# zobront/mythril

Hardware: AMD Instinct MI355X
Metric: candidate-assignment evals/sec (higher is better)
Workload: dtype u256 (u32 limbs); 1 GPU; C5 (BASELINE.json configs[4], per-GPU shard), exhaustive search; candidates_per_gpu_step=4194304, engine=jit (mwj_9cb5b0f4019c115a), jit_split=False, rccl_world=1, candidate_begin=0

## Files before the change

### mythril_amd/csrc/mw_alu.h

```cpp
#pragma once
#include <stdint.h>
#include <hip/hip_runtime.h>

#define MW_HD __host__ __device__ __attribute__((always_inline)) inline

#if defined(__HIP_DEVICE_COMPILE__)
#define MW_ANY(c) (__ballot(c) != 0ull)
#else
#define MW_ANY(c) (c)
#endif
#if defined(MW_DIV_NO_HINTS)
#define MW_RARE(c) (c)
#define MW_USUAL(c) (c)
#else
#define MW_RARE(c) __builtin_expect(!!(c), 0)
#define MW_USUAL(c) __builtin_expect(!!(c), 1)
#endif

namespace mw {
typedef uint32_t u32;
typedef uint64_t u64;

MW_HD u32 addc(u32 a, u32 b, u32& c) {
  u32 co;
// ... 392 lines not shown
#else
  const u32 n = y[7] ? 0u : y[6] ? 1u : y[5] ? 2u : y[4] ? 3u : y[3] ? 4u : y[2] ? 5u : y[1] ? 6u : 7u;
#pragma unroll
  for (int st = 0; st < 3; ++st) {
    const int m = 1 << st;
    const bool c = (n >> st) & 1u;
#pragma unroll
    for (int k = 7; k >= 0; --k) v[k] = c ? (k >= m ? v[k - m] : 0u) : v[k];
#pragma unroll
    for (int k = 15; k >= 0; --k) u[k] = c ? (k >= m ? u[k - m] : 0u) : u[k];
  }
#endif
  u32 w[9], lo[7], qq[8];
#pragma unroll
  for (int k = 0; k < 9; ++k) w[k] = u[7 + k];
#pragma unroll
  for (int k = 0; k < 7; ++k) lo[k] = u[k];
#pragma unroll
  for (int k = 0; k < 8; ++k) qq[k] = 0u;
#pragma unroll 1
  for (int it = 0; it < 8; ++it) {
    u32 qd = 0u;
    if (MW_ANY(w[8] != 0u || w[7] >= v[7])) {
      if (dc) dc->steps += 1u;
      qd = qdigit_est3(w[8], w[7], w[6], v[7], v[6]);
      u32 carry = 0, br = 0;
#pragma unroll
      for (int k = 0; k < 8; ++k) {
        const u64 p = (u64)qd * v[k] + carry;
        carry = (u32)(p >> 32);
        w[k] = subb(w[k], (u32)p, br);
      }
      u32 hi = w[8] - carry - br;
      while (MW_RARE(MW_ANY(hi != 0u))) {
        if (hi != 0u) {
          u32 c = 0;
#pragma unroll
          for (int k = 0; k < 8; ++k) w[k] = addc(w[k], v[k], c);
          hi += c;
          qd -= 1u;
        }
      }
      w[8] = 0u;
    }
#pragma unroll
    for (int k = 7; k > 0; --k) qq[k] = qq[k - 1];
    qq[0] = qd;
    if (it < 7) {
#pragma unroll
      for (int k = 8; k > 0; --k) w[k] = w[k - 1];
      w[0] = lo[6];
#pragma unroll
      for (int k = 6; k > 0; --k) lo[k] = lo[k - 1];
      lo[0] = 0u;
    }
  }
#pragma unroll
  for (int k = 0; k < 8; ++k) {
    q[k] = qq[k];
    u[k] = w[k];
    u[k + 8] = 0u;
  }
#if defined(MW_GEN_ROLLED_SHIFT)
#pragma unroll 1
  for (int st = 0; st < 7; ++st) {
    const bool c = n > (u32)st;
    if (!MW_ANY(c)) break;
#pragma unroll
    for (int k = 0; k < 7; ++k) u[k] = c ? u[k + 1] : u[k];
    u[7] = c ? 0u : u[7];
  }
#else
#pragma unroll
  for (int st = 0; st < 3; ++st) {
    const int m = 1 << st;
    const bool c = (n >> st) & 1u;
#pragma unroll
    for (int k = 0; k < 8; ++k) u[k] = c ? (k + m < 16 ? u[k + m] : 0u) : u[k];
  }
#endif
  copy8(r, u);
}

MW_HD void neg8(const u32 a[8], u32 r[8]) {
  u32 br = 0;
#pragma unroll
  for (int k = 0; k < 8; ++k) r[k] = subb(0u, a[k], br);
}
MW_HD void cneg8(u32 a[8], bool c, u32 w) {
  u32 br = 0;
#pragma unroll
  for (int k = 0; k < 8; ++k) {
    const u32 t = subb(0u, a[k], br);
    a[k] = c ? t : a[k];
  }
  canon(a, w);
}

MW_HD void wdiv(int kind, u32 x[8], u32 y[8], u32 w, u32 r[8], DivCount* dc = nullptr) {
  bool sa = false, sb = false;
  if (kind >= 2) {
    sa = signbit8(x, w);
    sb = signbit8(y, w);
    cneg8(x, sa, w);
    cneg8(y, sb, w);
  }
  const bool yz = is_zero8(y);
  y[0] |= yz ? 1u : 0u;
  u32 q[8];
  udivrem8(x, y, q, r, dc);
  if (yz) {
#pragma unroll
    for (int k = 0; k < 8; ++k) {
      q[k] = limb_mask(w, k);
      r[k] = x[k];
    }
  }
  switch (kind) {
    case 0:
      copy8(r, q);
      break;
    case 1:
      break;
    case 2:
      copy8(r, q);
      cneg8(r, sa != sb, w);
      break;
    case 3:
      cneg8(r, sa, w);
      break;
    default: {
      const bool uz = is_zero8(r);
      if (yz) y[0] = 0u;
      cneg8(y, sb, w);
      const bool negu = sa;
      cneg8(r, negu, w);
      const bool addt = !uz && (sa != sb);
      u32 c = 0;
#pragma unroll
      for (int k = 0; k < 8; ++k) {
        const u32 t = addc(r[k], y[k], c);
        r[k] = addt ? t : r[k];
      }
      break;
    }
  }
  canon(r, w);
}

MW_HD u32 n_sext(u32 a, u32 wfrom) {
  if (wfrom >= 32) return a;
  u32 s = (a >> (wfrom - 1)) & 1u;
  return s ? (a | ~nmask(wfrom)) : a;
}
MW_HD u32 n_div(int kind, u32 a, u32 b, u32 w) {
  u32 m = nmask(w);
  bool sa = false, sb = false;
  u32 x = a, y = b;
  if (kind >= 2) {
    sa = (a >> (w - 1)) & 1u;
    sb = (b >> (w - 1)) & 1u;
    x = sa ? ((0u - a) & m) : a;
    y = sb ? ((0u - b) & m) : b;
  }
  u32 q, rm;
  if (y == 0) {
    q = m;
    rm = x;
  } else {
    q = x / y;
    rm = x - q * y;
  }
  u32 r;
  switch (kind) {
    case 0: r = q; break;
    case 1: r = rm; break;
    case 2: r = (sa != sb) ? (0u - q) : q; break;
    case 3: r = sa ? (0u - rm) : rm; break;
    default: {
      if (rm == 0) r = 0;
      else if (!sa && !sb) r = rm;
      else if (sa && !sb) r = (0u - rm) + b;
      else if (!sa && sb) r = rm + b;
      else r = 0u - rm;
      break;
    }
  }
  return r & m;
}
MW_HD u32 n_shl(u32 a, u32 b, u32 w) { return b >= w ? 0u : ((a << b) & nmask(w)); }
MW_HD u32 n_lshr(u32 a, u32 b, u32 w) { return b >= w ? 0u : (a >> b); }
MW_HD u32 n_ashr(u32 a, u32 b, u32 w) {
  int32_t sa = (int32_t)n_sext(a, w);
  u32 s = b >= w ? 31u : b;
  return ((u32)(sa >> s)) & nmask(w);
}
MW_HD bool n_slt(u32 a, u32 b, u32 w) { return (int32_t)n_sext(a, w) < (int32_t)n_sext(b, w); }
MW_HD bool n_sle(u32 a, u32 b, u32 w) { return (int32_t)n_sext(a, w) <= (int32_t)n_sext(b, w); }
MW_HD bool n_umulno(u32 a, u32 b, u32 w) {
  u64 p = (u64)a * b;
  return w >= 32 ? (p >> 32) == 0 : (p >> w) == 0;
}

}
```

### mythril_amd/csrc/mw_jit.h

```cpp
#pragma once
#if defined(__HIP_DEVICE_COMPILE__)
#define MW_LEAF_KEY_FENCE(k) asm volatile("" : "+s"(k))
#endif
#include "mw_alu.h"
#include "mw_isa.h"
#include "mw_leaf.h"

namespace mw {
namespace jit {
MW_HD void xor8(const u32 x[8], const u32 y[8], u32 r[8]) {
#pragma unroll
  for (int k = 0; k < 8; ++k) r[k] = x[k] ^ y[k];
}

#if defined(MW_ABLATE_ADD)
#define add8(x, y, r) ((void)xor8(x, y, r), 0u)
#define sub8(x, y, r) ((void)xor8(x, y, r), 0u)
#endif
#if defined(MW_ABLATE_MUL)
#define mul8(x, y, r) xor8(x, y, r)
#endif
MW_HD void w_add(const u32 x[8], const u32 y[8], u32 w, u32 r[8]) { add8(x, y, r); canon(r, w); }
MW_HD void w_sub(const u32 x[8], const u32 y[8], u32 w, u32 r[8]) { sub8(x, y, r); canon(r, w); }
MW_HD void w_mul(const u32 x[8], const u32 y[8], u32 w, u32 r[8]) { mul8(x, y, r); canon(r, w); }
// ... 44 lines not shown
      "v_addc_co_u32_e64 %[c], %[s2], %[c], 0, %[s2]\n"
      "v_addc_co_u32_e64 %[c], %[s0], %[c], 0, %[s0]\n"
      "v_addc_co_u32_e64 %[c], %[s1], %[c], 0, %[s1]\n"
      : [p] "+v"(p), [c] "=&v"(c), [s0] "=&s"(s0), [s1] "=&s"(s1), [s2] "=&s"(s2)
      : [a0] "v"(a[0]), [a1] "v"(a[1]), [a2] "v"(a[2]), [a3] "v"(a[3]), [a4] "v"(a[4]), [b0] "v"(b[0]), [b1] "v"(b[1]), [b2] "v"(b[2]), [b3] "v"(b[3]), [b4] "v"(b[4]));
  r[4] = (u32)p;
  p = (p >> 32) | ((u64)c << 32);
  asm("v_mad_u64_u32 %[p], %[s0], %[a0], %[b5], %[p]\n"
      "v_mad_u64_u32 %[p], %[s1], %[a1], %[b4], %[p]\n"
      "v_mad_u64_u32 %[p], %[s2], %[a2], %[b3], %[p]\n"
      "v_addc_co_u32_e64 %[c], %[s0], 0, 0, %[s0]\n"
      "v_mad_u64_u32 %[p], %[s0], %[a3], %[b2], %[p]\n"
      "v_addc_co_u32_e64 %[c], %[s1], %[c], 0, %[s1]\n"
      "v_mad_u64_u32 %[p], %[s1], %[a4], %[b1], %[p]\n"
      "v_addc_co_u32_e64 %[c], %[s2], %[c], 0, %[s2]\n"
      "v_mad_u64_u32 %[p], %[s2], %[a5], %[b0], %[p]\n"
      "v_addc_co_u32_e64 %[c], %[s0], %[c], 0, %[s0]\n"
      "v_addc_co_u32_e64 %[c], %[s1], %[c], 0, %[s1]\n"
      "v_addc_co_u32_e64 %[c], %[s2], %[c], 0, %[s2]\n"
      : [p] "+v"(p), [c] "=&v"(c), [s0] "=&s"(s0), [s1] "=&s"(s1), [s2] "=&s"(s2)
      : [a0] "v"(a[0]), [a1] "v"(a[1]), [a2] "v"(a[2]), [a3] "v"(a[3]), [a4] "v"(a[4]), [a5] "v"(a[5]), [b0] "v"(b[0]), [b1] "v"(b[1]), [b2] "v"(b[2]), [b3] "v"(b[3]), [b4] "v"(b[4]), [b5] "v"(b[5]));
  r[5] = (u32)p;
  p = (p >> 32) | ((u64)c << 32);
  asm("v_mad_u64_u32 %[p], %[s0], %[a0], %[b6], %[p]\n"
      "v_mad_u64_u32 %[p], %[s1], %[a1], %[b5], %[p]\n"
      "v_mad_u64_u32 %[p], %[s2], %[a2], %[b4], %[p]\n"
      "v_mad_u64_u32 %[p], %[s0], %[a3], %[b3], %[p]\n"
      "v_mad_u64_u32 %[p], %[s1], %[a4], %[b2], %[p]\n"
      "v_mad_u64_u32 %[p], %[s2], %[a5], %[b1], %[p]\n"
      "v_mad_u64_u32 %[p], %[s0], %[a6], %[b0], %[p]\n"
      : [p] "+v"(p), [s0] "=&s"(s0), [s1] "=&s"(s1), [s2] "=&s"(s2)
      : [a0] "v"(a[0]), [a1] "v"(a[1]), [a2] "v"(a[2]), [a3] "v"(a[3]), [a4] "v"(a[4]), [a5] "v"(a[5]), [a6] "v"(a[6]), [b0] "v"(b[0]), [b1] "v"(b[1]), [b2] "v"(b[2]), [b3] "v"(b[3]), [b4] "v"(b[4]), [b5] "v"(b[5]), [b6] "v"(b[6]));
  r[6] = (u32)p;
  r[7] = (u32)(p >> 32) + a[0] * b[7] + a[1] * b[6] + a[2] * b[5] + a[3] * b[4] + a[4] * b[3] + a[5] * b[2] +
         a[6] * b[1] + a[7] * b[0];
#else
  mul8(a, b, r);
#endif
}
#if defined(MW_ABLATE_MUL)
#define mul8_cols(x, y, r) xor8(x, y, r)
#endif
MW_HD void w_mulv(const u32 x[8], const u32 y[8], u32 w, u32 r[8]) { mul8_cols(x, y, r); canon(r, w); }
MW_HD void w_and(const u32 x[8], const u32 y[8], u32 w, u32 r[8]) {
#pragma unroll
  for (int k = 0; k < 8; ++k) r[k] = x[k] & y[k];
  canon(r, w);
}
MW_HD void w_or(const u32 x[8], const u32 y[8], u32 w, u32 r[8]) {
#pragma unroll
  for (int k = 0; k < 8; ++k) r[k] = x[k] | y[k];
  canon(r, w);
}
MW_HD void w_xor(const u32 x[8], const u32 y[8], u32 w, u32 r[8]) {
#pragma unroll
  for (int k = 0; k < 8; ++k) r[k] = x[k] ^ y[k];
  canon(r, w);
}
MW_HD void w_not(const u32 x[8], u32 w, u32 r[8]) {
#pragma unroll
  for (int k = 0; k < 8; ++k) r[k] = ~x[k];
  canon(r, w);
}
#if defined(MW_ABLATE_SHIFT)
MW_HD void w_shl(const u32 x[8], const u32 y[8], u32 w, u32 r[8]) { xor8(x, y, r); }
MW_HD void w_lshr(const u32 x[8], const u32 y[8], u32 w, u32 r[8]) { xor8(x, y, r); }
MW_HD void w_ashr(const u32 x[8], const u32 y[8], u32 w, u32 r[8]) { xor8(x, y, r); }
#else
MW_HD void w_shl(const u32 x[8], const u32 y[8], u32 w, u32 r[8]) { wshl(x, y, w, r); canon(r, w); }
MW_HD void w_lshr(const u32 x[8], const u32 y[8], u32 w, u32 r[8]) { wlshr(x, y, w, r); canon(r, w); }
MW_HD void w_ashr(const u32 x[8], const u32 y[8], u32 w, u32 r[8]) { washr(x, y, w, r); canon(r, w); }
#endif
MW_HD void w_div(int kind, const u32 x[8], const u32 y[8], u32 w, u32 r[8], DivCount& dc) {
#if defined(MW_ABLATE_DIV)
  xor8(x, y, r);
  return;
#endif
  u32 a[8], b[8];
  copy8(a, x);
  copy8(b, y);
  wdiv(kind, a, b, w, r, &dc);
  canon(r, w);
}
MW_HD void w_ite(u32 c, const u32 x[8], const u32 y[8], u32 w, u32 r[8]) {
#pragma unroll
  for (int k = 0; k < 8; ++k) r[k] = c ? x[k] : y[k];
  canon(r, w);
}
MW_HD void w_shli(const u32 x[8], u32 imm, u32 w, u32 r[8]) { shl8(x, imm, r); canon(r, w); }
MW_HD void w_lshri(const u32 x[8], u32 imm, u32 w, u32 r[8]) { shr8(x, imm, 0u, r); canon(r, w); }
MW_HD void w_zextn(u32 v, u32 w, u32 r[8]) {
  zero8(r);
  r[0] = v;
  canon(r, w);
}
MW_HD void w_sext(const u32 x[8], u32 imm, u32 w, u32 r[8]) {
  copy8(r, x);
  sext8(r, imm);
  canon(r, w);
}
MW_HD void w_sextn(u32 v, u32 imm, u32 w, u32 r[8]) {
  zero8(r);
  r[0] = v;
  sext8(r, imm);
  canon(r, w);
}
MW_HD void w_insn(const u32 x[8], u32 v, u32 imm, u32 w, u32 r[8]) {
  u32 y[8];
  zero8(y);
  y[0] = v;
  shl8(y, imm, r);
#pragma unroll
  for (int k = 0; k < 8; ++k) r[k] |= x[k];
  canon(r, w);
}
MW_HD void w_mov(const u32 x[8], u32 w, u32 r[8]) {
  copy8(r, x);
  canon(r, w);
}

MW_HD u32 n_extractw(const u32 x[8], u32 imm, u32 w) {
  u32 r[8];
  shr8(x, imm, 0u, r);
  return r[0] & nmask(w);
}
MW_HD u32 n_ult(const u32 x[8], const u32 y[8]) { return ult8(x, y) ? 1u : 0u; }
MW_HD u32 n_ule(const u32 x[8], const u32 y[8]) { return ult8(y, x) ? 0u : 1u; }
MW_HD u32 n_scmp(const u32 x_[8], const u32 y_[8], u32 w, bool le) {
  u32 x[8], y[8];
#pragma unroll
  for (int k = 0; k < 8; ++k) {
    const int bit = (int)w - 1 - 32 * k;
    const u32 m = (bit >= 0 && bit < 32) ? (1u << bit) : 0u;
    x[k] = x_[k] ^ m;
    y[k] = y_[k] ^ m;
  }
  return (le ? !ult8(y, x) : ult8(x, y)) ? 1u : 0u;
}
MW_HD u32 n_eq(const u32 x[8], const u32 y[8]) { return eq8(x, y) ? 1u : 0u; }
MW_HD u32 n_umulno(const u32 x[8], const u32 y[8], u32 w) {
  u32 lo[8], hi[8];
  mulhi8(x, y, lo, hi);
  u32 ov = 0;
#pragma unroll
  for (int k = 0; k < 8; ++k) ov |= (lo[k] & ~limb_mask(w, k)) | hi[k];
  return ov ? 0u : 1u;
}
MW_HD u32 n_addc(const u32 x[8], const u32 y[8], u32 w) {
  u32 r[8];
  const u32 c = add8(x, y, r);
  u32 bit = 0;
#pragma unroll
  for (int k = 0; k < 8; ++k) {
    const int b = (int)w - 32 * k;
    bit |= (b >= 0 && b < 32) ? ((r[k] >> b) & 1u) : 0u;
  }
  return (w >= 256) ? c : bit;
}

MW_HD u32 nn_add(u32 a, u32 b, u32 w) { return (a + b) & nmask(w); }
MW_HD u32 nn_sub(u32 a, u32 b, u32 w) { return (a - b) & nmask(w); }
MW_HD u32 nn_mul(u32 a, u32 b, u32 w) { return (a * b) & nmask(w); }
MW_HD u32 nn_not(u32 a, u32 w) { return (~a) & nmask(w); }
MW_HD u32 nn_shli(u32 a, u32 imm, u32 w) { return (imm >= 32 ? 0u : (a << imm)) & nmask(w); }
MW_HD u32 nn_lshri(u32 a, u32 imm, u32 w) { return (imm >= 32 ? 0u : (a >> imm)) & nmask(w); }
MW_HD u32 nn_sext(u32 a, u32 imm, u32 w) { return n_sext(a, imm) & nmask(w); }
// ... 73 lines not shown
  do {                                                     \
    asm volatile("" : "+s"(ctl));                          \
    if (__builtin_expect((ctl & MW_JIT_NEVER) != 0u, 0))   \
      asm volatile("s_nop 0");                             \
  } while (0)
#else
#define JIT_SPLIT() ((void)ctl)
#endif

typedef bool (*body_fn)(const u32* __restrict__, u64, u64, bool, u32, u32*, u64, u64, DivCount&);

#define MW_JIT_FIRST 1u
#define MW_JIT_LAST 2u

#if !defined(MW_JIT_HOST)
template <body_fn BODY>
__device__ __attribute__((always_inline)) inline void search(const u32* __restrict__ pool, u64 seed, u64 begin,
                                                             u64 count, u64 chunk0, u32 flags,
                                                             u64* __restrict__ out_min, u64* __restrict__ counter,
                                                             u32* __restrict__ verdict, u32* __restrict__ alivebuf,
                                                             u32 stage) {
  const u64 base = begin + (chunk0 + blockIdx.x) * 256;
  if ((flags & MW_FLAG_STOP_AFTER_HIT) && stage == (MW_JIT_FIRST | MW_JIT_LAST)) {
    const u64 m = __hip_atomic_load(out_min, __ATOMIC_RELAXED, __HIP_MEMORY_SCOPE_AGENT);
    if (m <= base) return;
  }
  const u32 lane = threadIdx.x & 63u;
  const u64 cand = base + threadIdx.x;
  const bool valid = cand < begin + count;
  bool in = valid;
  if (!(stage & MW_JIT_FIRST) && valid) in = alivebuf[cand - begin] != 0u;
  DivCount dc;
  const bool ok = BODY(pool, seed, cand, in, flags, nullptr, 0, 0, dc);
  const u64 nvalid = (u64)__popcll(__ballot(valid));
  const bool counting = !(flags & MW_FLAG_NO_COUNT);
  counter += MW_CTR_STRIPE_WORDS * (1u + (blockIdx.x & (MW_CTR_STRIPES - 1u)));
  if (counting && lane == 0 && nvalid)
    add_div_counts(counter, dc, nvalid);
  if (!(stage & MW_JIT_LAST)) {
    if (valid) alivebuf[cand - begin] = ok ? 1u : 0u;
    return;
  }
  if (verdict && valid) verdict[cand - begin] = ok ? 1u : 0u;
  const u64 hit = __ballot(ok);
  if (hit) {
    const u32 first = (u32)__ffsll((unsigned long long)hit) - 1u;
    if (lane == first && cand < __hip_atomic_load(out_min, __ATOMIC_RELAXED, __HIP_MEMORY_SCOPE_AGENT))
      atomicMin((unsigned long long*)out_min, (unsigned long long)cand);
  }
  if (counting && lane == 0 && nvalid) atomicAdd((unsigned long long*)counter, (unsigned long long)nvalid);
}

#ifndef MW_JIT_WAVES
#define MW_JIT_WAVES 2
#endif
#define MW_JIT_KERNEL(NAME, SUFFIX, BODY, EARLY)                                                     \
  extern "C" __global__ __launch_bounds__(256, MW_JIT_WAVES) void NAME##SUFFIX(                      \
      const mw::u32* __restrict__ pool, mw::u64 seed, mw::u64 begin, mw::u64 count, mw::u64 chunk0,  \
      mw::u32 flags, mw::u64* __restrict__ out_min, mw::u64* __restrict__ counter,                   \
      mw::u32* __restrict__ verdict, mw::u32* __restrict__ alivebuf, mw::u32 stage) {                \
    mw::jit::search<BODY<EARLY>>(pool, seed, begin, count, chunk0, flags, out_min, counter, verdict, \
                                 alivebuf, stage);                                                   \
  }
#define MW_JIT_SIG(NAME, SIG) extern "C" __device__ const mw::u64 NAME##_sig = SIG;
#define MW_JIT_PART(NAME, K, N)                                \
  extern "C" __device__ const mw::u32 NAME##_part = K;         \
  extern "C" __device__ const mw::u32 NAME##_nparts = N;
#else
#define MW_JIT_KERNEL(NAME, SUFFIX, BODY, EARLY)
#define MW_JIT_SIG(NAME, SIG)
#define MW_JIT_PART(NAME, K, N)
#endif

#if defined(MW_JIT_HOST)
#define MW_JIT_HOST_ENTRY(NAME, BODY)                                                                \
  extern "C" int NAME##_host(const mw::u32* pool, mw::u64 seed, mw::u64 begin, mw::u64 count,        \
                             mw::u32 early, mw::u32* verdict, mw::u32* trace) {                      \
    for (mw::u64 i = 0; i < count; ++i) {                                                            \
      mw::DivCount ds;                                                                               \
      verdict[i] = (early ? BODY<true>(pool, seed, begin + i, true, 0u, trace, count, i, ds)             \
                          : BODY<false>(pool, seed, begin + i, true, 0u, trace, count, i, ds)) ? 1u : 0u; \
    }                                                                                                \
    return 0;                                                                                        \
  }
#else
#define MW_JIT_HOST_ENTRY(NAME, BODY)
#endif

}
}
```

### mythril_amd/jit.py

```python
from __future__ import annotations

import hashlib
import os
import subprocess
import sys
import tempfile
import time
from pathlib import Path
from typing import Dict, List, Optional, Sequence, Tuple

import numpy as np

from . import isa
from .compiler import Const, MInsn, Program, VReg, compile_program

ROOT = Path(__file__).resolve().parent.parent
CSRC = ROOT / "mythril_amd" / "csrc"
ARCH = os.environ.get("MW_OFFLOAD_ARCH", "gfx950")
HEADERS = ["mw_jit.h", "mw_alu.h", "mw_isa.h", "mw_leaf.h"]
M256 = (1 << 256) - 1
SPLIT_EVERY = 48
SPLIT_KIND = os.environ.get("MW_JIT_SPLIT", "branch")
CHECK_SYNC = os.environ.get("MW_JIT_CHECK_SYNC", "0") == "1"
CHECK_SYNC_EVERY = int(os.environ.get("MW_JIT_CHECK_SYNC_EVERY", "1"))
MUL_COLS = os.environ.get("MW_JIT_MUL_COLS", "1") == "1"
LDS_AHEAD = int(os.environ.get("MW_JIT_LDS_AHEAD", "16"))
LDS_AHEAD_W = int(os.environ.get("MW_JIT_LDS_AHEAD_W", "0"))
LDS_AHEAD_STOP = int(os.environ.get("MW_JIT_LDS_AHEAD_STOP", "500"))
LDS_REUSE = int(os.environ.get("MW_JIT_LDS_REUSE", "96"))
M32 = 0xFFFFFFFF

_WBIN = {"W_ADD": "w_add", "W_SUB": "w_sub", "W_MUL": "w_mul", "W_AND": "w_and", "W_OR": "w_or",
         "W_XOR": "w_xor", "W_SHL": "w_shl", "W_LSHR": "w_lshr", "W_ASHR": "w_ashr"}
_DIV = {"UDIV": 0, "UREM": 1, "SDIV": 2, "SREM": 3, "SMOD": 4}
_NBIN = {"N_ADD": "jit::nn_add({a}, {b}, {w})", "N_SUB": "jit::nn_sub({a}, {b}, {w})",
         "N_MUL": "jit::nn_mul({a}, {b}, {w})", "N_AND": "({a} & {b})", "N_OR": "({a} | {b})",
         "N_XOR": "({a} ^ {b})", "N_SHL": "n_shl({a}, {b}, {w})", "N_LSHR": "n_lshr({a}, {b}, {w})",
         "N_ASHR": "n_ashr({a}, {b}, {w})", "N_ULTN": "(u32)({a} < {b})", "N_ULEN": "(u32)({a} <= {b})",
         "N_SLTN": "(u32)n_slt({a}, {b}, {w})", "N_SLEN": "(u32)n_sle({a}, {b}, {w})",
         "N_EQN": "(u32)({a} == {b})", "N_UMULNON": "(u32)n_umulno({a}, {b}, {w})",
         "N_ADDCN": "jit::nn_addc({a}, {b}, {w})"}


def _cache_dir() -> Path:
    return Path(os.environ.get("MW_JIT_CACHE", str(ROOT / "build" / "jit")))


def signature(p: Program) -> int:
    h = 0xCBF29CE484222325
    for arr in (p.code, p.consts, p.leaves, p.pool):
        a = np.ascontiguousarray(arr, dtype=np.uint32)
        h = _fnv_words(h, a)
    return h


def _fnv_words(h: int, a: np.ndarray) -> int:
    b = a.astype("<u4").view(np.uint8)
    P = 0x100000001B3
    M = (1 << 64) - 1
    for x in b.tobytes():
        h = ((h ^ x) * P) & M
    return h


def interleave_conjuncts(insns: List[MInsn], k: int) -> List[MInsn]:
    if k <= 1:
        return list(insns)
    segs: List[List[MInsn]] = []
    cur: List[MInsn] = []
    tail: List[MInsn] = []
    for ins in insns:
        if ins.op == "END":
            tail.append(ins)
            continue
        cur.append(ins)
        if ins.op == "CHECK":
            segs.append(cur)
            cur = []
    if cur:
        segs.append(cur)
    out: List[MInsn] = []
    defined = set()
    for g in range(0, len(segs), k):
        group = segs[g:g + k]
        pos = [0] * len(group)
        left = sum(len(sg) for sg in group)
        while left:
            for j, sg in enumerate(group):
                if pos[j] >= len(sg):
                    continue
                ins = sg[pos[j]]
                if any(isinstance(s_, VReg) and s_.id not in defined for s_ in ins.srcs):
                    continue
                out.append(ins)
                if ins.dst is not None:
                    defined.add(ins.dst.id)
                pos[j] += 1
                left -= 1
    return out + tail


class _Gen:

    def __init__(self, p: Program, name: str, fence_first: bool = False, lds_leaves: int = 0,
                 insns: Optional[List[MInsn]] = None, interleave: int = 1, mul_cols: Optional[bool] = None):
        self.fence_first = fence_first
        self.mul_cols = MUL_COLS if mul_cols is None else mul_cols
        self.p = p
        self.insns = interleave_conjuncts(p.machine_ir() if insns is None else insns, interleave)
        uses: Dict[int, int] = {}
        defs: Dict[int, int] = {}
        for ins in self.insns:
            if ins.op == "LEAF_W":
                defs[ins.dst.id] = ins.imm
            for s_ in ins.srcs:
                if isinstance(s_, VReg) and s_.id in defs:
                    uses[s_.id] = uses.get(s_.id, 0) + 1
        hot = sorted(uses, key=lambda v: -uses[v])[:lds_leaves]
        self.lds_slot: Dict[int, int] = {v: k for k, v in enumerate(hot)}
        self.pre: List[str] = []
        self.nl = 0
        self.name = name
        self.wconst: Dict[int, str] = {}
        self.lines: List[str] = []
        self.since_split = 0
        self.nf = 0
        self.put_at: Dict[int, int] = {}
        self.line_w: List[int] = []
        self.nchecks = 0
        self.last_reload: Dict[int, Tuple[str, int]] = {}

    def W(self, s) -> str:
        if isinstance(s, Const):
            v = s.value & M256
            n = self.wconst.get(v)
            if n is None:
                n = f"k{len(self.wconst)}"
                self.wconst[v] = n
            return n
        if s.cls != "W":
            raise ValueError("N register in a W operand")
        slot = self.lds_slot.get(s.id)
        if slot is not None:
            last = self.last_reload.get(s.id)
            if LDS_REUSE and last is not None and len(self.lines) - last[1] <= LDS_REUSE:
                return last[0]
            self.nl += 1
            self.last_reload[s.id] = (f"L{self.nl}", len(self.lines))
            self.pre.append(("R", f"u32 L{self.nl}[8]; jit::lds_get8({slot}u, L{self.nl});", s.id))
            return f"L{self.nl}"
        return f"v{s.id}"

    def N(self, s) -> str:
        if isinstance(s, Const):
            return f"{s.value & M32:#x}u"
        if s.cls != "N":
            raise ValueError("W register in an N operand")
        return f"n{s.id}"

    def leaf(self, li: int, dst: str):
        L = [int(x) for x in self.p.leaves[li * isa.LEAF_WORDS:(li + 1) * isa.LEAF_WORDS]]
        w, kind, lid, shift, bits, poff, _inrow, stride = L
        return (f"leaf_fields({w}u, {kind}u, {lid:#x}u, {shift}u, {bits}u, {poff}u, {stride}u, "
                f"pool, seed, cand, {dst});")

    def emit(self, ins) -> None:
        n0 = len(self.lines)
        self._emit(ins)
        self.line_w.extend([0] * (len(self.lines) - len(self.line_w)))
        if len(self.lines) > n0:
            self.line_w[-1] = insn_weight(ins)

    def _emit(self, ins) -> None:
        op, w, d, S, imm = ins.op, ins.width, ins.dst, ins.srcs, ins.imm
        self.since_split += 1
        if self.since_split > SPLIT_EVERY and op != "CHECK":
            self.lines.append("JIT_SPLIT();")
            self.since_split = 0
        if op == "END":
            return
        shape = isa.SHAPES[op]
        A = [self.W(s) if c == "W" else self.N(s) for s, c in zip(S, shape[1])]
        out = self.lines.append
        for x in self.pre:
            out(x)
        self.pre = []
        fence = getattr(ins, "remat", False)
        if fence or (self.fence_first and S and op not in ("CHECK", "STORE_W", "STORE_N")):
            for j, (s, c) in enumerate(zip(S, shape[1])):
                if not fence and j > 0:
                    break
                if isinstance(s, VReg):
                    self.nf += 1
                    if c == "W":
                        out(f"u32 f{self.nf}[8]; jit::fence8({A[j]}, f{self.nf});")
                        A[j] = f"f{self.nf}"
                    else:
                        out(f"const u32 f{self.nf} = jit::fence1({A[j]});")
                        A[j] = f"f{self.nf}"
        dn = None
        if d is not None:
            dn = f"v{d.id}" if d.cls == "W" else f"n{d.id}"
        if op == "CHECK":
            self.nchecks += 1
            sync = CHECK_SYNC and self.nchecks % CHECK_SYNC_EVERY == 0
            tail = "{ JIT_SPLIT(); JIT_SYNC(); }" if sync else "JIT_SPLIT();"
            out(f"alive = jit::check(alive, {A[0]}); if (EARLY) {{ if (jit::none(alive)) break; }} else {tail}")
            self.since_split = 0
        elif op == "LEAF_W" and d.id in self.lds_slot:
            out(f"{{ u32 t_[8]; {self.leaf(imm, 't_')} jit::lds_put8({self.lds_slot[d.id]}u, t_); }}")
            self.put_at[d.id] = len(self.lines)
        elif op == "LEAF_W":
            out(f"u32 {dn}[8]; {self.leaf(imm, dn)}")
        elif op == "LEAF_N":
            out(f"u32 {dn}; {{ u32 t_[8]; {self.leaf(imm, 't_')} {dn} = t_[0]; }}")
        elif op in ("STORE_W", "STORE_N"):
            row = self.p.trace_map[-imm - 1][0]
            if op == "STORE_W":
                out(f"jit::tstore(trace, tstride, tidx, {row}u, {A[0]}, 8);")
            else:
                out(f"{{ const u32 t_ = {A[0]}; jit::tstore(trace, tstride, tidx, {row}u, &t_, 1); }}")
        elif op == "MOV_W":
            out(f"u32 {dn}[8]; jit::w_mov({A[0]}, {w}u, {dn});")
        elif op == "MOV_N":
            out(f"const u32 {dn} = {A[0]};")
        elif op == "W_MUL" and self.mul_cols and all(isinstance(s, VReg) for s in S):
            out(f"u32 {dn}[8]; jit::w_mulv({A[0]}, {A[1]}, {w}u, {dn});")
        elif op in _WBIN:
            out(f"u32 {dn}[8]; jit::{_WBIN[op]}({A[0]}, {A[1]}, {w}u, {dn});")
        elif op.startswith("W_") and op[2:] in _DIV:
            out(f"u32 {dn}[8]; jit::w_div({_DIV[op[2:]]}, {A[0]}, {A[1]}, {w}u, {dn}, dsteps);")
        elif op == "W_NOT":
            out(f"u32 {dn}[8]; jit::w_not({A[0]}, {w}u, {dn});")
        elif op == "W_ITE":
            out(f"u32 {dn}[8]; jit::w_ite({A[2]}, {A[0]}, {A[1]}, {w}u, {dn});")
        elif op == "W_SHLI":
            out(f"u32 {dn}[8]; jit::w_shli({A[0]}, {imm}u, {w}u, {dn});")
        elif op == "W_LSHRI":
            out(f"u32 {dn}[8]; jit::w_lshri({A[0]}, {imm}u, {w}u, {dn});")
        elif op == "W_ZEXTN":
            out(f"u32 {dn}[8]; jit::w_zextn({A[0]}, {w}u, {dn});")
        elif op == "W_SEXT":
            out(f"u32 {dn}[8]; jit::w_sext({A[0]}, {imm}u, {w}u, {dn});")
        elif op == "W_SEXTN":
            out(f"u32 {dn}[8]; jit::w_sextn({A[0]}, {imm}u, {w}u, {dn});")
        elif op == "W_INSN":
            out(f"u32 {dn}[8]; jit::w_insn({A[0]}, {A[1]}, {imm}u, {w}u, {dn});")
        elif op == "N_EXTRACTW":
            out(f"const u32 {dn} = jit::n_extractw({A[0]}, {imm}u, {w}u);")
        elif op == "N_ULT":
            out(f"const u32 {dn} = jit::n_ult({A[0]}, {A[1]});")
        elif op == "N_ULE":
            out(f"const u32 {dn} = jit::n_ule({A[0]}, {A[1]});")
        elif op in ("N_SLT", "N_SLE"):
            le = "true" if op == "N_SLE" else "false"
            out(f"const u32 {dn} = jit::n_scmp({A[0]}, {A[1]}, {w}u, {le});")
        elif op == "N_EQ":
            out(f"const u32 {dn} = jit::n_eq({A[0]}, {A[1]});")
        elif op == "N_UMULNO":
            out(f"const u32 {dn} = jit::n_umulno({A[0]}, {A[1]}, {w}u);")
        elif op == "N_ADDC":
            out(f"const u32 {dn} = jit::n_addc({A[0]}, {A[1]}, {w}u);")
        elif op in _NBIN:
            out(f"const u32 {dn} = " + _NBIN[op].format(a=A[0], b=A[1], w=f"{w}u") + ";")
        elif op.startswith("N_") and op[2:] in _DIV:
            out(f"const u32 {dn} = n_div({_DIV[op[2:]]}, {A[0]}, {A[1]}, {w}u);")
        elif op == "N_NOT":
            out(f"const u32 {dn} = jit::nn_not({A[0]}, {w}u);")
        elif op == "N_ITE":
            out(f"const u32 {dn} = {A[2]} ? {A[0]} : {A[1]};")
        elif op == "N_SHLI":
            out(f"const u32 {dn} = jit::nn_shli({A[0]}, {imm}u, {w}u);")
        elif op == "N_LSHRI":
            out(f"const u32 {dn} = jit::nn_lshri({A[0]}, {imm}u, {w}u);")
        elif op == "N_SEXT":
            out(f"const u32 {dn} = jit::nn_sext({A[0]}, {imm}u, {w}u);")
        else:
            raise ValueError(f"jit: no emitter for {op}")

    def _place_reloads(self) -> List[str]:
        if LDS_AHEAD <= 0 and LDS_AHEAD_W <= 0:
            return [x[1] if isinstance(x, tuple) else x for x in self.lines]
        before: Dict[int, List[str]] = {}
        rest: List[Tuple[int, str]] = []
        for i, x in enumerate(self.lines):
            if isinstance(x, tuple):
                floor = self.put_at.get(x[2], -1) + 1
                if LDS_AHEAD_W > 0:
                    j, acc = i, 0
                    while j > floor and acc < LDS_AHEAD_W:
                        j -= 1
                        acc += self.line_w[j]
                elif LDS_AHEAD_STOP < (1 << 30):
                    j = i
                    while j > floor and i - j < LDS_AHEAD and self.line_w[j - 1] < LDS_AHEAD_STOP:
                        j -= 1
                else:
                    j = max(i - LDS_AHEAD, floor)
                before.setdefault(j, []).append(x[1])
            else:
                rest.append((i, x))
        out: List[str] = []
        pend = sorted(before)
        k = 0
        for i, x in rest:
            while k < len(pend) and pend[k] <= i:
                out += before[pend[k]]
                k += 1
            out.append(x)
        while k < len(pend):
            out += before[pend[k]]
            k += 1
        return out

    def body(self) -> str:
        for ins in self.insns:
            self.emit(ins)
        self.lines = self._place_reloads()
        head = [f"template <bool EARLY>",
                f"MW_HD bool {self.name}_body(const u32* __restrict__ pool, u64 seed, u64 cand, bool alive,",
                f"                             u32 ctl, u32* __restrict__ trace, u64 tstride, u64 tidx,",
                f"                             DivCount& dsteps) {{"]
        consts = []
        for v, n in self.wconst.items():
            limbs = ", ".join(f"{(v >> (32 * k)) & M32:#x}u" for k in range(8))
            consts.append(f"  const u32 {n}[8] = {{{limbs}}};")
        return "\n".join(head + consts + ["  do {"] + ["    " + x for x in self.lines] +
                         ["  } while (0);", "  return alive;", "}"])


PART_WEIGHT = 110_000
_WEIGHT = {"W_UDIV": 900, "W_UREM": 900, "W_SDIV": 950, "W_SREM": 950, "W_SMOD": 950, "W_MUL": 110,
           "W_SHL": 45, "W_LSHR": 45, "W_ASHR": 45, "LEAF_W": 200, "LEAF_N": 100, "N_ULT": 25, "N_ULE": 25,
           "N_SLT": 30, "N_SLE": 30, "N_EQ": 16, "N_UMULNO": 150, "N_ADDC": 12}


def insn_weight(ins: MInsn) -> int:
    w = _WEIGHT.get(ins.op)
    if w is not None:
        return w
    return 10 if ins.op.startswith("W_") else 3


def split_ssa(p: Program, part_weight: int = PART_WEIGHT) -> List[List[MInsn]]:
    ssa = [i for i in p.machine_ir() if i.op != "END"]
    n = len(ssa)
    total = sum(insn_weight(i) for i in ssa)
    if total <= part_weight * 1.25 or n < 2:
        return [p.machine_ir()]
    defs: Dict[int, int] = {}
    last: Dict[int, int] = {}
    for i, ins in enumerate(ssa):
        if ins.dst is not None:
            defs[ins.dst.id] = i
        for s_ in ins.srcs:
            if isinstance(s_, VReg):
                last[s_.id] = i
    delta = [0] * (n + 2)
    for vid, d in defs.items():
        if ssa[d].op.startswith("LEAF"):
            continue
        l = last.get(vid, d)
        if l > d:
            delta[d + 1] += 1
            delta[l + 1] -= 1
    cuts, acc, cross = [], 0, 0
    target = total / max(2, round(total / part_weight))
    for b in range(1, n):
        cross += delta[b]
        acc += insn_weight(ssa[b - 1])
        if acc >= target and ssa[b - 1].op == "CHECK" and cross == 0:
            cuts.append(b)
            acc = 0
    if not cuts:
        return [p.machine_ir()]
    bounds = [0] + cuts + [n]
    parts = []
    for a, b in zip(bounds, bounds[1:]):
        seg = ssa[a:b]
        inside = {ins.dst.id for ins in seg if ins.dst is not None}
        need, stack = set(), [s_.id for ins in seg for s_ in ins.srcs if isinstance(s_, VReg)]
        while stack:
            v = stack.pop()
            if v in inside or v in need:
                continue
            need.add(v)
            stack.extend(s_.id for s_ in ssa[defs[v]].srcs if isinstance(s_, VReg))
        pre = [ssa[defs[v]] for v in sorted(need, key=lambda v: defs[v])]
        parts.append(pre + seg + [MInsn("END")])
    return parts


def generate(progs: Sequence[Program], names: Sequence[str], variants: str = "xe",
             fence_first: bool = False, lds_leaves: int = 0,
             parts: Optional[Sequence[Tuple[List[MInsn], int, int]]] = None, interleave: int = 1,
             mul_cols: Optional[bool] = None) -> str:
    out = ["// generated by mythril_amd/jit.py: specialised witness-search kernels"]
    if lds_leaves:
        out.append(f"#define MW_JIT_LDS_SLOTS {lds_leaves}")
    out += ['#include "mw_jit.h"', "using namespace mw;", ""]
    if SPLIT_KIND == "sched_barrier":
        out += ["#if defined(__HIP_DEVICE_COMPILE__)", "#undef JIT_SPLIT",
                "#define JIT_SPLIT() __builtin_amdgcn_sched_barrier(0)", "#endif", ""]
    if CHECK_SYNC:
        out += ["#if defined(__HIP_DEVICE_COMPILE__)", "#define JIT_SYNC() __syncthreads()", "#else",
                "#define JIT_SYNC() ((void)0)", "#endif", ""]
    done = set()
    for k, (p, name) in enumerate(zip(progs, names)):
        if name in done:
            continue
        done.add(name)
        if not p.machine_ir():
            raise ValueError("program has no SSA machine IR (compiled by an older compiler?)")
        part = parts[k] if parts else None
        out.append(f"// program {name}: {p.n_insn} bytecode insns, {p.ops_per_eval} u32 ops/eval"
                   + (f", part {part[1]} of {part[2]}" if part else ""))
        out.append(_Gen(p, name, fence_first, lds_leaves, part[0] if part else None, interleave, mul_cols).body())
        out.append(f"MW_JIT_SIG({name}, {signature(p):#x}ull)")
        if part:
            out.append(f"MW_JIT_PART({name}, {part[1]}u, {part[2]}u)")
        if "x" in variants:
            out.append(f"MW_JIT_KERNEL({name}, _x, {name}_body, false)")
        if "e" in variants:
            out.append(f"MW_JIT_KERNEL({name}, _e, {name}_body, true)")
        out.append(f"MW_JIT_HOST_ENTRY({name}, {name}_body)")
        out.append("")
    return "\n".join(out)


def kernel_name(p: Program) -> str:
    return f"mwj_{signature(p):016x}"


def _hipcc() -> str:
    return "/opt/rocm/bin/hipcc" if os.path.exists("/opt/rocm/bin/hipcc") else "hipcc"


def _key(src: str, flags: Sequence[str]) -> str:
    h = hashlib.sha256(src.encode())
    h.update(" ".join(flags).encode())
    for hd in HEADERS:
        h.update((CSRC / hd).read_bytes())
    return h.hexdigest()[:24]


DEVICE_FLAGS = ["--genco", f"--offload-arch={ARCH}", "-O3", "-std=c++17", "-Wno-unused-variable"]
HOST_FLAGS = ["-O1", "-std=c++17", "-fPIC", "-shared", "-D__HIP_PLATFORM_AMD__", "-DMW_JIT_HOST",
              "-Wno-unused-variable"]


_USED: set = set()


def prune_cache(keep: Optional[set] = None) -> int:
    keep = _USED if keep is None else keep
    n = 0
    for f in _cache_dir().glob("*"):
        if f not in keep:
            f.unlink()
            n += 1
    return n


def _compile(src: str, flags: Sequence[str], suffix: str, ext: str) -> Tuple[Path, float]:
    cache = _cache_dir()
    cache.mkdir(parents=True, exist_ok=True)
    out = cache / f"{_key(src, flags)}{suffix}"
    _USED.add(out)
    if out.exists():
        return out, 0.0
    t0 = time.perf_counter()
    with tempfile.TemporaryDirectory() as td:
        f = Path(td) / f"k{ext}"
        f.write_text(src)
        tmp = Path(td) / ("out" + suffix)
        proc = subprocess.Popen([_hipcc(), *flags, f"-I{CSRC}", str(f), "-o", str(tmp)],
                                stdout=subprocess.PIPE, stderr=subprocess.PIPE, text=True)
        while True:
            try:
                _, err = proc.communicate(timeout=30)
                break
            except subprocess.TimeoutExpired:
                print(f"[jit] compiling {len(src) // 1024} KiB of HIP for {ARCH}: "
                      f"{time.perf_counter() - t0:.0f} s", file=sys.stderr, flush=True)
        if proc.returncode != 0:
            raise RuntimeError(f"jit compile failed:\n{err[-4000:]}")
        os.replace(tmp, out)
    return out, time.perf_counter() - t0


def is_cached(progs: Sequence[Program], variants: str = "xe", waves: int = 2, lds_leaves: int = 0,
              interleave: int = 1, mul_cols: Optional[bool] = None) -> bool:
    names = [kernel_name(p) for p in progs]
    src = generate(progs, names, variants, lds_leaves=lds_leaves, interleave=interleave, mul_cols=mul_cols)
    return (_cache_dir() / f"{_key(src, _device_flags(waves))}.hsaco").exists()


def compile_device(progs: Sequence[Program], variants: str = "xe", fence_first: bool = False,
                   waves: int = 2, lds_leaves: int = 0, interleave: int = 1,
                   mul_cols: Optional[bool] = None) -> Tuple[bytes, List[str], float]:
# ... 139 lines not shown
```

Before: 250.9 million evals/s.

## Specialise JIT div and mul kernels on statically inferred operand limb bounds

Adds a value-range analysis over the SSA machine IR that bounds each 256-bit value's bit width and tracks known-nonzero values. The code generator uses these bounds to emit templated narrow-limb multiply and divide routines in place of full 8-limb ones. The divide keeps a wave-uniform runtime check that falls back to the full routine if a bound is violated. This cuts multiply and long-division work when operands are provably small, at the cost of extra template instantiations, more code size, and reliance on the analysis being correct.

Result: faster. 258.2 million evals/s, median of 6 (+2.9%).

```diff
diff --git a/mythril_amd/csrc/mw_alu.h b/mythril_amd/csrc/mw_alu.h
--- a/mythril_amd/csrc/mw_alu.h
+++ b/mythril_amd/csrc/mw_alu.h
@@ -498,6 +498,69 @@
   copy8(r, u);
 }
 
+template <int NX, int NY>
+MW_HD void udivrem8_nb(const u32 x[8], const u32 y[8], u32 q[8], u32 r[8], DivCount* dc = nullptr) {
+  static_assert(NX >= 0 && NX <= 8 && NY >= 1 && NY <= 8, "limb bounds");
+  u32 over = 0u;
+#pragma unroll
+  for (int k = NX; k < 8; ++k) over |= x[k];
+#pragma unroll
+  for (int k = NY; k < 8; ++k) over |= y[k];
+  if (MW_RARE(MW_ANY(over != 0u || y[NY - 1] == 0u))) {
+    udivrem8(x, y, q, r, dc);
+    return;
+  }
+  if (NY == 8) {
+    if (dc) dc->full += 1u;
+    zero8(q);
+#pragma unroll
+    for (int k = 0; k < 8; ++k) r[k] = k < NX ? x[k] : 0u;
+    return;
+  }
+  if (NY == 1) {
+    u32 xs[8];
+#pragma unroll
+    for (int k = 0; k < 8; ++k) xs[k] = k < NX ? x[k] : 0u;
+    udivrem8_short(xs, y[0], q, r);
+    if (dc) dc->shrt += 1u;
+    return;
+  }
+  if (dc) dc->gen += 1u;
+  constexpr int D = NY < 2 ? 2 : (NY > 7 ? 7 : NY);
+  u32 u[10];
+#pragma unroll
+  for (int k = 0; k < 10; ++k) u[k] = k < NX ? x[k] : 0u;
+  zero8(q);
+#pragma unroll
+  for (int j = NX - D; j >= 0; --j) {
+    if (MW_ANY(u[j + D] != 0u || u[j + D - 1] >= y[D - 1])) {
+      if (dc) dc->steps += 1u;
+      u32 qd = qdigit_est3(u[j + D], u[j + D - 1], u[j + D - 2], y[D - 1], y[D - 2]);
+      u32 carry = 0, br = 0;
+#pragma unroll
+      for (int k = 0; k < D; ++k) {
+        const u64 p = (u64)qd * y[k] + carry;
+        carry = (u32)(p >> 32);
+        u[j + k] = subb(u[j + k], (u32)p, br);
+      }
+      u32 hi = u[j + D] - carry - br;
+      while (MW_RARE(MW_ANY(hi != 0u))) {
+        if (hi != 0u) {
+          u32 c = 0;
+#pragma unroll
+          for (int k = 0; k < D; ++k) u[j + k] = addc(u[j + k], y[k], c);
+          hi += c;
+          qd -= 1u;
+        }
+      }
+      u[j + D] = 0u;
+      q[j] = qd;
+    }
+  }
+#pragma unroll
+  for (int k = 0; k < 8; ++k) r[k] = k < D ? u[k] : 0u;
+}
+
 MW_HD void neg8(const u32 a[8], u32 r[8]) {
   u32 br = 0;
 #pragma unroll
@@ -551,6 +614,57 @@
       cneg8(y, sb, w);
       const bool negu = sa;
       cneg8(r, negu, w);
+      const bool addt = !uz && (sa != sb);
+      u32 c = 0;
+#pragma unroll
+      for (int k = 0; k < 8; ++k) {
+        const u32 t = addc(r[k], y[k], c);
+        r[k] = addt ? t : r[k];
+      }
+      break;
+    }
+  }
+  canon(r, w);
+}
+
+template <int NX, int NY>
+MW_HD void wdiv_nb(int kind, u32 x[8], u32 y[8], u32 w, u32 r[8], DivCount* dc = nullptr) {
+  bool sa = false, sb = false;
+  if (kind >= 2) {
+    sa = signbit8(x, w);
+    sb = signbit8(y, w);
+    cneg8(x, sa, w);
+    cneg8(y, sb, w);
+  }
+  const bool yz = is_zero8(y);
+  y[0] |= yz ? 1u : 0u;
+  u32 q[8];
+  udivrem8_nb<NX, NY>(x, y, q, r, dc);
+  if (yz) {
+#pragma unroll
+    for (int k = 0; k < 8; ++k) {
+      q[k] = limb_mask(w, k);
+      r[k] = x[k];
+    }
+  }
+  switch (kind) {
+    case 0:
+      copy8(r, q);
+      break;
+    case 1:
+      break;
+    case 2:
+      copy8(r, q);
+      cneg8(r, sa != sb, w);
+      break;
+    case 3:
+      cneg8(r, sa, w);
+      break;
+    default: {
+      const bool uz = is_zero8(r);
+      if (yz) y[0] = 0u;
+      cneg8(y, sb, w);
+      cneg8(r, sa, w);
       const bool addt = !uz && (sa != sb);
       u32 c = 0;
 #pragma unroll
diff --git a/mythril_amd/csrc/mw_jit.h b/mythril_amd/csrc/mw_jit.h
--- a/mythril_amd/csrc/mw_jit.h
+++ b/mythril_amd/csrc/mw_jit.h
@@ -150,6 +150,30 @@
   wdiv(kind, a, b, w, r, &dc);
   canon(r, w);
 }
+template <int NX, int NY>
+MW_HD void w_div_nb(int kind, const u32 x[8], const u32 y[8], u32 w, u32 r[8], DivCount& dc) {
+#if defined(MW_ABLATE_DIV)
+  xor8(x, y, r);
+  return;
+#endif
+  u32 a[8], b[8];
+  copy8(a, x);
+  copy8(b, y);
+  wdiv_nb<NX, NY>(kind, a, b, w, r, &dc);
+  canon(r, w);
+}
+template <int NA, int NB>
+MW_HD void w_mul_nb(const u32 x[8], const u32 y[8], u32 w, u32 r[8]) {
+  u32 a[8], b[8];
+#pragma unroll
+  for (int k = 0; k < 8; ++k) {
+    a[k] = k < NA ? x[k] : 0u;
+    b[k] = k < NB ? y[k] : 0u;
+  }
+  if (NA <= NB) mul8(a, b, r);
+  else mul8(b, a, r);
+  canon(r, w);
+}
 MW_HD void w_ite(u32 c, const u32 x[8], const u32 y[8], u32 w, u32 r[8]) {
 #pragma unroll
   for (int k = 0; k < 8; ++k) r[k] = c ? x[k] : y[k];
@@ -389,6 +413,20 @@
                           : BODY<false>(pool, seed, begin + i, true, 0u, trace, count, i, ds)) ? 1u : 0u; \
     }                                                                                                \
     return 0;                                                                                        \
+  }                                                                                                  \
+   \
+  extern "C" int NAME##_host_dc(const mw::u32* pool, mw::u64 seed, mw::u64 begin, mw::u64 count,     \
+                                mw::u64* out) {                                                      \
+    for (int k = 0; k < 4; ++k) out[k] = 0;                                                          \
+    for (mw::u64 i = 0; i < count; ++i) {                                                            \
+      mw::DivCount ds;                                                                               \
+      (void)BODY<false>(pool, seed, begin + i, true, 0u, nullptr, count, i, ds);                     \
+      out[0] += ds.steps;                                                                            \
+      out[1] += ds.full;                                                                             \
+      out[2] += ds.shrt;                                                                             \
+      out[3] += ds.gen;                                                                              \
+    }                                                                                                \
+    return 0;                                                                                        \
   }
 #else
 #define MW_JIT_HOST_ENTRY(NAME, BODY)
diff --git a/mythril_amd/jit.py b/mythril_amd/jit.py
--- a/mythril_amd/jit.py
+++ b/mythril_amd/jit.py
@@ -28,6 +28,8 @@
 LDS_AHEAD_W = int(os.environ.get("MW_JIT_LDS_AHEAD_W", "0"))
 LDS_AHEAD_STOP = int(os.environ.get("MW_JIT_LDS_AHEAD_STOP", "500"))
 LDS_REUSE = int(os.environ.get("MW_JIT_LDS_REUSE", "96"))
+RANGES = os.environ.get("MW_JIT_RANGES", "1") != "0"
+RANGES_MUL = True
 M32 = 0xFFFFFFFF
 
 _WBIN = {"W_ADD": "w_add", "W_SUB": "w_sub", "W_MUL": "w_mul", "W_AND": "w_and", "W_OR": "w_or",
@@ -100,14 +102,113 @@
     return out + tail
 
 
+def value_bounds(insns: Sequence[MInsn], p: Optional[Program] = None) -> Dict[int, int]:
+    b: Dict[int, int] = {}
+    nz: set = set()
+
+    def bound(s, width):
+        if isinstance(s, Const):
+            return (s.value & M256).bit_length()
+        if s.cls != "W":
+            return 32
+        return b.get(s.id, width if 0 < width <= 256 else 256)
+
+    def nonzero(s, width):
+        if isinstance(s, Const):
+            return (s.value & ((1 << width) - 1)) != 0
+        return s.id in nz
+
+    for ins in insns:
+        d = ins.dst
+        if d is None or d.cls != "W":
+            continue
+        op, S = ins.op, ins.srcs
+        w = ins.width if 0 < ins.width <= 256 else 256
+        B = [bound(s, w) for s in S]
+        r = w
+        if op == "LEAF_W" and p is not None:
+            r = int(p.leaves[ins.imm * isa.LEAF_WORDS])
+        elif op == "MOV_W":
+            r = B[0]
+            if B[0] <= w and nonzero(S[0], w):
+                nz.add(d.id)
+        elif op == "W_AND":
+            r = min(B)
+        elif op in ("W_OR", "W_XOR"):
+            r = max(B)
+            if op == "W_OR" and any(bb <= w and nonzero(s, w) for s, bb in zip(S, B)):
+                nz.add(d.id)
+        elif op == "W_ADD":
+            r = max(B) + 1
+        elif op == "W_MUL":
+            r = 0 if 0 in B else B[0] + B[1]
+        elif op == "W_SHLI":
+            r = B[0] + ins.imm if B[0] else 0
+        elif op == "W_LSHRI":
+            r = max(B[0] - ins.imm, 0)
+        elif op == "W_LSHR":
+            r = B[0]
+        elif op == "W_ASHR":
+            r = B[0] if B[0] < w else w
+        elif op == "W_ITE":
+            r = max(B[0], B[1])
+            if all(bb <= w and nonzero(s, w) for s, bb in zip(S[:2], B[:2])):
+                nz.add(d.id)
+        elif op == "W_ZEXTN":
+            r = 32
+        elif op == "W_INSN":
+            r = max(B[0], ins.imm + 32)
+        elif op in ("W_UDIV", "W_UREM", "W_SDIV", "W_SREM", "W_SMOD"):
+            unsigned = op in ("W_UDIV", "W_UREM") or (B[0] < w and B[1] < w)
+            if not unsigned:
+                r = w
+            elif op in ("W_UDIV", "W_SDIV"):
+                r = B[0] if nonzero(S[1], w) else w
+            else:
+                r = min(B[0], B[1]) if nonzero(S[1], w) else B[0]
+        b[d.id] = max(0, min(r, w))
+    return b
+
+
+def _limbs(bits: int) -> int:
+    return (bits + 31) // 32
+
+
+def _site_bounds(ins: MInsn, bounds: Dict[int, int]) -> Tuple[int, int]:
+    w = ins.width if 0 < ins.width <= 256 else 256
+    out = []
+    for s in ins.srcs[:2]:
+        bits = (s.value & M256).bit_length() if isinstance(s, Const) else bounds.get(s.id, w)
+        out.append(_limbs(min(bits, w)))
+    return out[0], out[1]
+
+
+def range_sites(p: Program, insns: Optional[Sequence[MInsn]] = None) -> Dict[str, Dict[Tuple[int, int], int]]:
+    insns = p.machine_ir() if insns is None else insns
+    bounds = value_bounds(insns, p)
+    out: Dict[str, Dict[Tuple[int, int], int]] = {"div": {}, "mul": {}}
+    for ins in insns:
+        if ins.op.startswith("W_") and ins.op[2:] in _DIV:
+            nx, ny = _site_bounds(ins, bounds)
+            key, kind = (nx, max(ny, 1)), "div"
+        elif ins.op == "W_MUL" and all(isinstance(s, VReg) for s in ins.srcs):
+            key, kind = _site_bounds(ins, bounds), "mul"
+        else:
+            continue
+        out[kind][key] = out[kind].get(key, 0) + 1
+    return out
+
+
 class _Gen:
 
     def __init__(self, p: Program, name: str, fence_first: bool = False, lds_leaves: int = 0,
-                 insns: Optional[List[MInsn]] = None, interleave: int = 1, mul_cols: Optional[bool] = None):
+                 insns: Optional[List[MInsn]] = None, interleave: int = 1, mul_cols: Optional[bool] = None,
+                 ranges: Optional[bool] = None):
         self.fence_first = fence_first
         self.mul_cols = MUL_COLS if mul_cols is None else mul_cols
         self.p = p
         self.insns = interleave_conjuncts(p.machine_ir() if insns is None else insns, interleave)
+        self.bounds = value_bounds(self.insns, p) if (RANGES if ranges is None else ranges) else None
         uses: Dict[int, int] = {}
         defs: Dict[int, int] = {}
         for ins in self.insns:
@@ -225,11 +326,17 @@
         elif op == "MOV_N":
             out(f"const u32 {dn} = {A[0]};")
         elif op == "W_MUL" and self.mul_cols and all(isinstance(s, VReg) for s in S):
-            out(f"u32 {dn}[8]; jit::w_mulv({A[0]}, {A[1]}, {w}u, {dn});")
+            na, nb = _site_bounds(ins, self.bounds) if self.bounds is not None and RANGES_MUL else (8, 8)
+            if min(na, nb) < 8:
+                out(f"u32 {dn}[8]; jit::w_mul_nb<{na}, {nb}>({A[0]}, {A[1]}, {w}u, {dn});")
+            else:
+                out(f"u32 {dn}[8]; jit::w_mulv({A[0]}, {A[1]}, {w}u, {dn});")
         elif op in _WBIN:
             out(f"u32 {dn}[8]; jit::{_WBIN[op]}({A[0]}, {A[1]}, {w}u, {dn});")
         elif op.startswith("W_") and op[2:] in _DIV:
-            out(f"u32 {dn}[8]; jit::w_div({_DIV[op[2:]]}, {A[0]}, {A[1]}, {w}u, {dn}, dsteps);")
+            nx, ny = _site_bounds(ins, self.bounds) if self.bounds is not None else (8, 8)
+            nb = f"_nb<{nx}, {max(ny, 1)}>" if min(nx, ny) < 8 else ""
+            out(f"u32 {dn}[8]; jit::w_div{nb}({_DIV[op[2:]]}, {A[0]}, {A[1]}, {w}u, {dn}, dsteps);")
         elif op == "W_NOT":
             out(f"u32 {dn}[8]; jit::w_not({A[0]}, {w}u, {dn});")
         elif op == "W_ITE":
@@ -394,7 +501,7 @@
 def generate(progs: Sequence[Program], names: Sequence[str], variants: str = "xe",
              fence_first: bool = False, lds_leaves: int = 0,
              parts: Optional[Sequence[Tuple[List[MInsn], int, int]]] = None, interleave: int = 1,
-             mul_cols: Optional[bool] = None) -> str:
+             mul_cols: Optional[bool] = None, ranges: Optional[bool] = None) -> str:
     out = ["// generated by mythril_amd/jit.py: specialised witness-search kernels"]
     if lds_leaves:
         out.append(f"#define MW_JIT_LDS_SLOTS {lds_leaves}")
@@ -415,7 +522,7 @@
         part = parts[k] if parts else None
         out.append(f"// program {name}: {p.n_insn} bytecode insns, {p.ops_per_eval} u32 ops/eval"
                    + (f", part {part[1]} of {part[2]}" if part else ""))
-        out.append(_Gen(p, name, fence_first, lds_leaves, part[0] if part else None, interleave, mul_cols).body())
+        out.append(_Gen(p, name, fence_first, lds_leaves, part[0] if part else None, interleave, mul_cols, ranges).body())
         out.append(f"MW_JIT_SIG({name}, {signature(p):#x}ull)")
         if part:
             out.append(f"MW_JIT_PART({name}, {part[1]}u, {part[2]}u)")
```
